# CESSProject/DeOSS

Measured on AMD Instinct MI355X. Metric: device-resident GiB/s hashed to Merkle root; 1/2/4/8 MI355X scaling, higher is better.
Workload: dtype u32; 1 GPU; BASELINE configs[1]: 1 object of 8 GiB (8589934592 B) in 1 chunk-range shard(s) of 8 GiB, chunk 33554432 B (256 leaves); object_bytes=8589934592, chunk=33554432, leaves=256, parallelism=single GPU

## Files before the change

deoss_amd/csrc/merkle_kernels.hpp:

```cpp
#pragma once
#include "quad_ring.hpp"
#include "sha256_gfx950.hpp"

namespace dm {

constexpr int kBlock = 256;
constexpr int kLeafFuseMax = 8;
constexpr int kReduceTile = 512;

struct LeafArgs {
    const uint8_t* base;
    uint64_t pitch;
    uint64_t leaf_len;
    uint64_t last_len;
    const uint64_t* addrs;
    const uint64_t* lens;
    uint64_t nleaves;
    uint64_t byte_off;
    uint64_t byte_end;
    uint32_t* state;
    uint8_t* digests;
    uint8_t* level_out;
    uint32_t fuse_levels;
};
// ... 398 lines not shown
    const uint64_t first = (uint64_t)blockIdx.x * kPairLeaves;
    const uint64_t i = first + c;
    const LeafView v = leaf_view<TABLE>(a, i);
    const uint64_t NB = wave_max_u64(v.nb);
    if (producer) {
        Blk cur;
        if (v.nb > 0 && !lane_b) cur = load_block<ALIGNED>(v.p);
        for (uint64_t b = 0; b < NB; b++) {
            if (b < v.nb) {
                uint32_t w[16];
                block_words(cur, w);
                if (b + 1 < v.nb && !lane_b) cur = load_block<ALIGNED>(v.p + 64 * (b + 1));
                uint4 (*kw)[kLatLeaves] = ring[b % kLatRing];
#pragma unroll
                for (int q = 0; q < 16; q++) {
                    uint32_t u[4];
#pragma unroll
                    for (int j = 0; j < 4; j++) {
                        const int t = 4 * q + j;
                        uint32_t wt;
                        if (t < 16) {
                            wt = w[t];
                        } else {
                            wt = ssig1(w[(t - 2) & 15]) + w[(t - 7) & 15] + ssig0(w[(t - 15) & 15]) + w[t & 15];
                            w[t & 15] = wt;
                        }
                        u[j] = lane_b ? 0u : kSha256K[t] + wt;
                    }
                    kw[q][lane] = make_uint4(u[0], u[1], u[2], u[3]);
                }
            }
            __syncthreads();
        }
        __syncthreads();
    } else {
        const uint32_t sh1 = lane_b ? 2 : 6, sh2 = lane_b ? 13 : 11, sh3 = lane_b ? 22 : 25;
        const uint32_t msk = lane_b ? 0u : ~0u;
        uint32_t st0[8];
        if (v.active) load_or_init_state(a, i, st0);
        else init_state(st0);
        uint32_t x[4];
#pragma unroll
        for (int k = 0; k < 4; k++) x[k] = lane_b ? st0[k] : st0[4 + k];
        __syncthreads();
        for (uint64_t b = 0; b < NB; b++) {
            if (b < v.nb) pair_rounds_from_kw(x, ring[b % kLatRing], lane, sh1, sh2, sh3, msk, lane_b);
            __syncthreads();
        }
        uint32_t st[8];
#pragma unroll
        for (int k = 0; k < 4; k++) {
            const uint32_t other = dpp_swap_pairs(x[k]);
            st[k] = lane_b ? x[k] : other;
            st[4 + k] = lane_b ? other : x[k];
        }
        if (v.active && !lane_b) {
            leaf_epilogue<ALIGNED>(a, i, v, st);
#pragma unroll
            for (int k = 0; k < 8; k++) lds_a[c][k] = st[k];
        }
    }
    if (a.fuse_levels == 0) return;
    __syncthreads();
    const uint32_t cnt = (uint32_t)((a.nleaves - first) < kPairLeaves ? (a.nleaves - first) : kPairLeaves);
    uint32_t (*res)[8];
    const uint32_t out_cnt = lds_reduce(lds_a, lds_b, cnt, a.fuse_levels, &res);
    if (threadIdx.x < out_cnt) {
        uint32_t o8[8];
#pragma unroll
        for (int k = 0; k < 8; k++) o8[k] = res[threadIdx.x][k];
        const uint64_t o = (uint64_t)blockIdx.x * (kPairLeaves >> a.fuse_levels) + threadIdx.x;
        store_digest(a.level_out + 32 * o, o8);
    }
}

constexpr int kQuadLeaves = 8;
constexpr int kQuadBlocks = 8;
constexpr int kQuadFuseMax = 3;
constexpr int kQuadRow = kQuadLeaves;
constexpr size_t kQuadLdsBytes = sizeof(uint4) * kLatRing * 16 * kQuadBlocks * kQuadRow + 4 * 8 * kQuadLeaves +
                                 4 * 8 * (kQuadLeaves / 2);
static_assert(4 * kQuadLdsBytes <= (160u << 10), "four compact K1Q workgroups must fit a CU's LDS");

#define DM_QS_HEAD(X4, X5, X6)                                                                   \
    "v_alignbit_b32 %[r], %[" X4 "], %[" X4 "], %[sh]\n\t"                                      \
    "v_bitop3_b32 %[f], %[" X4 "], %[" X5 "], %[msk] bitop3:0x1e\n\t"                          \
    "v_bitop3_b32 %[f], %[f], %[" X6 "], %[" X5 "] bitop3:0xca\n\t"                             \
    "v_xor_b32_dpp %[s], %[r], %[r] quad_perm:[1,2,0,3] row_mask:0xf bank_mask:0xf\n\t"
#define DM_QS_SIGMA "v_xor_b32_dpp %[s], %[r], %[s] quad_perm:[2,0,1,3] row_mask:0xf bank_mask:0xf\n\t"
#define DM_QS_STEP_Q(X4, X5, X6, X7, H, HN, VN, QP)                                             \
    DM_QS_HEAD(X4, X5, X6)                                                                       \
    "v_sub_u32_dpp %[" X6 "], %[" VN "], %[" X6 "] quad_perm:" QP " row_mask:0xf bank_mask:0x3\n\t" \
    DM_QS_SIGMA                                                                                  \
    "v_sub_u32_dpp %[" HN "], %[" X4 "], %[" X6 "] row_ror:8 row_mask:0xf bank_mask:0xf\n\t"    \
    "v_add3_u32 %[" X7 "], %[s], %[f], %[" H "]\n\t"
#define DM_QS_STEP(X4, X5, X6, X7, H, HN, VN) DM_QS_STEP_Q(X4, X5, X6, X7, H, HN, VN, "[0,1,2,3]")
#define DM_QS_STEP_A(X4, X5, X6, X7, H, HN)                                                     \
    DM_QS_HEAD(X4, X5, X6)                                                                       \
    DM_QS_SIGMA                                                                                  \
    "v_sub_u32_dpp %[" HN "], %[" X4 "], %[" X6 "] row_ror:8 row_mask:0xf bank_mask:0xf\n\t"    \
    "v_add3_u32 %[" X7 "], %[s], %[f], %[" H "]\n\t"
#define DM_QS_STEP_END(X4, X5, X6, X7, H)                                                       \
    DM_QS_HEAD(X4, X5, X6)                                                                       \
    DM_QS_SIGMA                                                                                  \
    "v_add3_u32 %[" X7 "], %[s], %[f], %[" H "]\n\t"
#define DM_QS_STEPS4V(V0, V1, V2, V3)                                                          \
    DM_QS_STEP("a", "b", "c", "d", "h", "g", V0) DM_QS_STEP("d", "a", "b", "c", "g", "h", V1)   \
    DM_QS_STEP("c", "d", "a", "b", "h", "g", V2) DM_QS_STEP("b", "c", "d", "a", "g", "h", V3)
#define DM_QS_ALIGN_MIS ".p2align 3\n\t.if %[mis]\n\ts_nop 0\n\t.endif\n\t"
#define DM_QS_PROLOGUE(V) DM_QS_PROLOGUE_AT(V, DM_QS_ALIGN_MIS, "[0,1,2,3]")
#define DM_QS_PROLOGUE_AT(V, ALIGN, QP)                                                           \
    "s_nop 1\n\t" ALIGN                                                                          \
    "v_sub_u32_dpp %[d], %[" V "], %[d] quad_perm:" QP " row_mask:0xf bank_mask:0x3\n\t"         \
    "v_sub_u32_dpp %[h], %[b], %[d] row_ror:8 row_mask:0xf bank_mask:0xf\n\t"
#define DM_QS_RESTORE_A(P, X) "v_mov_b32_dpp %[" P "], %[" X "] quad_perm:[0,1,2,3] row_mask:0xf bank_mask:0xc\n\t"
#define DM_QS_GROUP0(V0, V1, V2, V3)                                                             \
    DM_QS_STEP("a", "b", "c", "d", "h", "g", V0) DM_QS_RESTORE_A("d", "x3")                      \
    DM_QS_STEP("d", "a", "b", "c", "g", "h", V1) DM_QS_RESTORE_A("c", "x2")                      \
    DM_QS_STEP("c", "d", "a", "b", "h", "g", V2) DM_QS_STEP("b", "c", "d", "a", "g", "h", V3)
#define DM_QS_FF(X, P, BANKS) "v_add_u32_dpp %[" X "], %[" P "], %[" X "] quad_perm:[0,1,2,3] row_mask:0xf bank_mask:" BANKS "\n\t"
#define DM_QS_TAIL(V0, V1, V2)                                                                   \
    DM_QS_STEP("a", "b", "c", "d", "h", "g", V0) DM_QS_STEP("d", "a", "b", "c", "g", "h", V1)   \
    DM_QS_STEP("c", "d", "a", "b", "h", "g", V2) DM_QS_STEP_A("b", "c", "d", "a", "g", "h")      \
    DM_QS_FF("x3", "d", "0x3") DM_QS_FF("x2", "c", "0x3") DM_QS_FF("x1", "b", "0x3")             \
    DM_QS_FF("x0", "a", "0x3")                                                                   \
    DM_QS_STEP_A("a", "b", "c", "d", "h", "g") DM_QS_STEP_END("d", "a", "b", "c", "g")           \
    DM_QS_FF("x0", "a", "0xc") DM_QS_FF("x1", "b", "0xc") DM_QS_FF("x3", "d", "0xc")             \
    DM_QS_FF("x2", "c", "0xc")
#define DM_QS_STEPS4Q(V0, Q0, V1, Q1, V2, Q2, V3, Q3)                                          \
    DM_QS_STEP_Q("a", "b", "c", "d", "h", "g", V0, Q0) DM_QS_STEP_Q("d", "a", "b", "c", "g", "h", V1, Q1) \
    DM_QS_STEP_Q("c", "d", "a", "b", "h", "g", V2, Q2) DM_QS_STEP_Q("b", "c", "d", "a", "g", "h", V3, Q3)
#define DM_QS_GROUP0Q(V0, Q0, V1, Q1, V2, Q2, V3, Q3)                                          \
    DM_QS_STEP_Q("a", "b", "c", "d", "h", "g", V0, Q0) DM_QS_RESTORE_A("d", "x3")              \
    DM_QS_STEP_Q("d", "a", "b", "c", "g", "h", V1, Q1) DM_QS_RESTORE_A("c", "x2")              \
    DM_QS_STEP_Q("c", "d", "a", "b", "h", "g", V2, Q2) DM_QS_STEP_Q("b", "c", "d", "a", "g", "h", V3, Q3)
#define DM_QS_TAILQ(V0, Q0, V1, Q1, V2, Q2)                                                     \
    DM_QS_STEP_Q("a", "b", "c", "d", "h", "g", V0, Q0) DM_QS_STEP_Q("d", "a", "b", "c", "g", "h", V1, Q1) \
    DM_QS_STEP_Q("c", "d", "a", "b", "h", "g", V2, Q2) DM_QS_STEP_A("b", "c", "d", "a", "g", "h") \
    DM_QS_FF("x3", "d", "0x3") DM_QS_FF("x2", "c", "0x3") DM_QS_FF("x1", "b", "0x3")             \
    DM_QS_FF("x0", "a", "0x3")                                                                   \
    DM_QS_STEP_A("a", "b", "c", "d", "h", "g") DM_QS_STEP_END("d", "a", "b", "c", "g")           \
    DM_QS_FF("x0", "a", "0xc") DM_QS_FF("x1", "b", "0xc") DM_QS_FF("x3", "d", "0xc")             \
    DM_QS_FF("x2", "c", "0xc")
#define DM_QS_OUT                                                                                \
    : [a] "+v"(p0), [b] "+v"(p1), [c] "+v"(p2), [d] "+v"(p3), [h] "+v"(h), [g] "+v"(g),           \
      [x0] "+v"(x[0]), [x1] "+v"(x[1]), [x2] "+v"(x[2]), [x3] "+v"(x[3]), [r] "=&v"(r_),          \
      [f] "=&v"(f_), [s] "=&v"(s_)
#define DM_QS_OPS DM_QS_OUT : [mis] "i"(MIS ? 1 : 0), [sh] "v"(sh.x), [msk] "v"(msk), [v0] "v"(v0), [v1] "v"(v1), [v2] "v"(v2), [v3] "v"(v3)

template <bool MIS, class KW>
__device__ __forceinline__ void quad_block_skewed(uint32_t (&x)[4], KW kw, uint3 sh, uint32_t msk) {
    uint32_t p0 = x[0], p1 = x[1], p2 = x[2], p3 = x[3], h = 0, g = 0, r_, f_, s_;
    uint4 q = kw(0), nq = kw(1);
    {
        const uint32_t v0 = q.x, v1 = 0, v2 = 0, v3 = 0;
        asm volatile(DM_QS_PROLOGUE("v0") DM_QS_OPS);
    }
#pragma unroll
    for (int grp = 0; grp < 16; grp++) {
        const uint4 nnq = grp + 2 < 16 ? kw(grp + 2) : nq;
        const uint32_t v0 = q.y, v1 = q.z, v2 = q.w, v3 = nq.x;
        if (grp == 0) {
            asm volatile(DM_QS_ALIGN_MIS DM_QS_GROUP0("v0", "v1", "v2", "v3") DM_QS_OPS);
        } else if (grp < 15) {
            asm volatile(DM_QS_ALIGN_MIS DM_QS_STEPS4V("v0", "v1", "v2", "v3") DM_QS_OPS);
        } else {
            asm volatile(DM_QS_ALIGN_MIS DM_QS_TAIL("v0", "v1", "v2") DM_QS_OPS);
        }
        q = nq;
        nq = nnq;
    }
}

constexpr int kLgkmWait0 = 0xC07F;

#define DM_QS_HNB(HN, A, B, BANKS) "v_sub_u32_dpp %[" HN "], %[" A "], %[" B "] row_ror:8 row_mask:0xf bank_mask:" BANKS "\n\t"
#define DM_QS_ADDB(D, A, B, BANKS) "v_add_u32_dpp %[" D "], %[" A "], %[" B "] quad_perm:[0,1,2,3] row_mask:0xf bank_mask:" BANKS "\n\t"
#define DM_QS_MOVB(D, S, BANKS) "v_mov_b32_dpp %[" D "], %[" S "] quad_perm:[0,1,2,3] row_mask:0xf bank_mask:" BANKS "\n\t"
#define DM_QS_KWN(X6, S, N) "v_sub_u32_dpp %[" X6 "], %[" N "], %[" S "] quad_perm:[0,0,0,0] row_mask:0xf bank_mask:0x3\n\t"
#define DM_QS_ADD3(X7, H) "v_add3_u32 %[" X7 "], %[s], %[f], %[" H "]\n\t"
#define DM_QS_LINKQ(V0, Q0, V1, Q1, V2, Q2, N0, N1, N2)                                          \
    DM_QS_STEP_Q("a", "b", "c", "d", "h", "g", V0, Q0) DM_QS_STEP_Q("d", "a", "b", "c", "g", "h", V1, Q1) \
    DM_QS_STEP_Q("c", "d", "a", "b", "h", "g", V2, Q2)                                           \
    DM_QS_ADDB("x1", "x1", "b", "0xc") DM_QS_ADDB("x3", "x3", "d", "0x3")                        \
                                            \
    DM_QS_HEAD("b", "c", "d") DM_QS_KWN("d", "x3", N0) DM_QS_SIGMA                               \
    DM_QS_HNB("h", "x1", "d", "0x3") DM_QS_HNB("h", "b", "d", "0xc") DM_QS_ADD3("a", "g")        \
    DM_QS_ADDB("b", "x1", "b", "0x3") DM_QS_ADDB("c", "x2", "c", "0x3")                          \
    DM_QS_HNB("g", "a", "c", "0xc") DM_QS_ADDB("x0", "x0", "a", "0xc")                           \
    DM_QS_ADDB("a", "a", "x0", "0x3") DM_QS_MOVB("x2", "c", "0x3")                               \
                                                            \
    DM_QS_HEAD("a", "b", "c") DM_QS_KWN("c", "c", N1) DM_QS_SIGMA                                \
    DM_QS_HNB("g", "x0", "c", "0x3") DM_QS_ADD3("d", "h")                                        \
    DM_QS_ADDB("x3", "x3", "d", "0xc") DM_QS_MOVB("x1", "b", "0x3") DM_QS_MOVB("x0", "a", "0x3") \
                                           \
    DM_QS_HEAD("d", "a", "b") DM_QS_KWN("b", "b", N2) DM_QS_SIGMA                                \
    DM_QS_HNB("h", "x3", "b", "0x3") DM_QS_HNB("h", "d", "x1", "0xc") DM_QS_ADD3("c", "g")       \
    DM_QS_ADDB("x2", "x2", "c", "0xc") DM_QS_MOVB("a", "x0", "0xc") DM_QS_MOVB("d", "x3", "0xc") \
    DM_QS_MOVB("c", "x2", "0xc")
#define DM_QS_BODYQ                                                                              \
    DM_QS_STEPS4Q("q01", "[1,1,1,1]", "q02", "[1,1,1,1]", "q03", "[1,1,1,1]", "q00", "[2,2,2,2]") \
    DM_QS_STEPS4Q("q01", "[2,2,2,2]", "q02", "[2,2,2,2]", "q03", "[2,2,2,2]", "q00", "[3,3,3,3]") \
    DM_QS_STEPS4Q("q01", "[3,3,3,3]", "q02", "[3,3,3,3]", "q03", "[3,3,3,3]", "q10", "[0,0,0,0]") \
    DM_QS_STEPS4Q("q11", "[0,0,0,0]", "q12", "[0,0,0,0]", "q13", "[0,0,0,0]", "q10", "[1,1,1,1]") \
    DM_QS_STEPS4Q("q11", "[1,1,1,1]", "q12", "[1,1,1,1]", "q13", "[1,1,1,1]", "q10", "[2,2,2,2]") \
    DM_QS_STEPS4Q("q11", "[2,2,2,2]", "q12", "[2,2,2,2]", "q13", "[2,2,2,2]", "q10", "[3,3,3,3]") \
    DM_QS_STEPS4Q("q11", "[3,3,3,3]", "q12", "[3,3,3,3]", "q13", "[3,3,3,3]", "q20", "[0,0,0,0]") \
    DM_QS_STEPS4Q("q21", "[0,0,0,0]", "q22", "[0,0,0,0]", "q23", "[0,0,0,0]", "q20", "[1,1,1,1]") \
    DM_QS_STEPS4Q("q21", "[1,1,1,1]", "q22", "[1,1,1,1]", "q23", "[1,1,1,1]", "q20", "[2,2,2,2]") \
    DM_QS_STEPS4Q("q21", "[2,2,2,2]", "q22", "[2,2,2,2]", "q23", "[2,2,2,2]", "q20", "[3,3,3,3]") \
    DM_QS_STEPS4Q("q21", "[3,3,3,3]", "q22", "[3,3,3,3]", "q23", "[3,3,3,3]", "q30", "[0,0,0,0]") \
    DM_QS_STEPS4Q("q31", "[0,0,0,0]", "q32", "[0,0,0,0]", "q33", "[0,0,0,0]", "q30", "[1,1,1,1]") \
    DM_QS_STEPS4Q("q31", "[1,1,1,1]", "q32", "[1,1,1,1]", "q33", "[1,1,1,1]", "q30", "[2,2,2,2]") \
    DM_QS_STEPS4Q("q31", "[2,2,2,2]", "q32", "[2,2,2,2]", "q33", "[2,2,2,2]", "q30", "[3,3,3,3]")
#define DM_QS_FILLQ                                                                              \
    DM_QS_PROLOGUE_AT("q00", DM_QS_ALIGN_MIS, "[0,0,0,0]")                                       \
    DM_QS_GROUP0Q("q01", "[0,0,0,0]", "q02", "[0,0,0,0]", "q03", "[0,0,0,0]", "q00", "[1,1,1,1]")
#define DM_QS_CONTQ                                                                              \
    DM_QS_ALIGN_MIS                                                                              \
    DM_QS_STEP_Q("c", "d", "a", "b", "h", "g", "q03", "[0,0,0,0]") DM_QS_STEP_Q("b", "c", "d", "a", "g", "h", "q00", "[1,1,1,1]")
#define DM_QS_ENDLINKQ DM_QS_LINKQ("q31", "[3,3,3,3]", "q32", "[3,3,3,3]", "q33", "[3,3,3,3]", "n0", "n1", "n2")
#define DM_QS_ENDTAILQ DM_QS_TAILQ("q31", "[3,3,3,3]", "q32", "[3,3,3,3]", "q33", "[3,3,3,3]")
#define DM_QS_STATE [a] "+v"(P[0]), [b] "+v"(P[1]), [c] "+v"(P[2]), [d] "+v"(P[3]),              \
                    [x0] "+v"(x[0]), [x1] "+v"(x[1]), [x2] "+v"(x[2]), [x3] "+v"(x[3]),           \
                    [r] "=&v"(r_), [f] "=&v"(f_), [s] "=&v"(s_)
#define DM_QS_KIN [mis] "i"(MIS ? 1 : 0), [sh] "v"(sh.x), [msk] "v"(msk),                        \
                  [q00] "v"(K[0].x), [q01] "v"(K[0].y), [q02] "v"(K[0].z), [q03] "v"(K[0].w),     \
                  [q10] "v"(K[1].x), [q11] "v"(K[1].y), [q12] "v"(K[1].z), [q13] "v"(K[1].w),     \
                  [q20] "v"(K[2].x), [q21] "v"(K[2].y), [q22] "v"(K[2].z), [q23] "v"(K[2].w),     \
                  [q30] "v"(K[3].x), [q31] "v"(K[3].y), [q32] "v"(K[3].z), [q33] "v"(K[3].w)

template <bool MIS, int K8>
__device__ __forceinline__ void quad_block_regs(uint32_t (&x)[4], uint32_t (&P)[4], uint32_t& h, uint32_t& g,
                                                const uint4 (&K)[4], const uint4& N, uint3 sh, uint32_t msk) {
    uint32_t r_, f_, s_;
    if constexpr (K8 == 0) {
        asm volatile(DM_QS_FILLQ DM_QS_BODYQ DM_QS_ENDLINKQ
                     : DM_QS_STATE, [h] "=&v"(h), [g] "=&v"(g)
                     : DM_QS_KIN, [n0] "v"(N.x), [n1] "v"(N.y), [n2] "v"(N.z));
    } else if constexpr (K8 < kQuadBlocks - 1) {
        asm volatile(DM_QS_CONTQ DM_QS_BODYQ DM_QS_ENDLINKQ
                     : DM_QS_STATE, [h] "+v"(h), [g] "+v"(g)
                     : DM_QS_KIN, [n0] "v"(N.x), [n1] "v"(N.y), [n2] "v"(N.z));
    } else {
        asm volatile(DM_QS_CONTQ DM_QS_BODYQ DM_QS_ENDTAILQ
                     : DM_QS_STATE, [h] "+v"(h), [g] "+v"(g)
                     : DM_QS_KIN);
    }
}

template <int G, int ROW, bool MIS, int K8 = 0>
__device__ __forceinline__ void quad_stage_blocks(uint32_t (&x)[4], uint32_t (&P)[4], uint32_t& h, uint32_t& g,
                                                  uint4 (&S)[3][4], const uint4* kw, uint3 sh, uint32_t msk) {
    __builtin_amdgcn_s_waitcnt(kLgkmWait0);
    if constexpr (K8 + 2 < kQuadBlocks) {
#pragma unroll
        for (int t = 0; t < 4; t++) S[(K8 + 2) % 3][t] = kw[(K8 + 2) * ROW + 4 * t * G];
    }
    quad_block_regs<MIS, K8>(x, P, h, g, S[K8 % 3], S[(K8 + 1) % 3][0], sh, msk);
    if constexpr (K8 + 1 < kQuadBlocks) quad_stage_blocks<G, ROW, MIS, K8 + 1>(x, P, h, g, S, kw, sh, msk);
}
template <int G, int ROW, bool MIS>
__device__ __forceinline__ void quad_stage_regs(uint32_t (&x)[4], const uint4* kw, uint3 sh, uint32_t msk) {
    uint4 S[3][4];
    uint32_t P[4] = {x[0], x[1], x[2], x[3]}, h, g;
#pragma unroll
    for (int k = 0; k < 2; k++) {
#pragma unroll
        for (int t = 0; t < 4; t++) S[k][t] = kw[k * ROW + 4 * t * G];
    }
    quad_stage_blocks<G, ROW, MIS>(x, P, h, g, S, kw, sh, msk);
}

constexpr int kQuadWideRing = quad_ring::kWideDepth;
constexpr int kQuadSets = quad_ring::kSets;
template <int G, int ROW, int K8, bool FILL, bool TAIL, bool LOAD>
__device__ __forceinline__ void quad_xstage_block(uint32_t (&x)[4], uint32_t (&P)[4], uint32_t& h, uint32_t& g,
                                                  uint4 (&S)[kQuadSets][4], const uint4* src, uint3 sh, uint32_t msk) {
    static_assert((LOAD || !quad_ring::block_prefetches(K8, true)) && (!TAIL || !quad_ring::block_links(K8, true)) &&
                      !(FILL && TAIL) && quad_ring::prefetch_of(K8).block == (K8 + quad_ring::kAhead) % kQuadBlocks,
                  "only the last stage of a run skips a load or drains: quad_ring.hpp");
    __builtin_amdgcn_s_waitcnt(kLgkmWait0);
    if constexpr (LOAD) {
        constexpr quad_ring::BlockRef pf = quad_ring::prefetch_of(K8);
#pragma unroll
        for (int t = 0; t < 4; t++) S[quad_ring::set_of(K8 + quad_ring::kAhead)][t] = src[pf.block * ROW + 4 * t * G];
    }
    quad_block_regs<false, FILL ? 0 : TAIL ? kQuadBlocks - 1 : 1>(x, P, h, g, S[quad_ring::set_of(K8)],
                                                                 S[quad_ring::set_of(K8 + 1)][0], sh, msk);
}
template <int G, int ROW>
__device__ __forceinline__ uint32_t quad_run_xstage(uint32_t (&x)[4], const uint4* colp, uint32_t slot, uint64_t n,
                                                    uint3 sh, uint32_t msk) {
    uint4 S[kQuadSets][4];
    uint32_t P[4] = {x[0], x[1], x[2], x[3]}, h, g;
    const uint4* cur = colp + slot * 16 * G;
#pragma unroll
    for (int k = 0; k < quad_ring::kAhead; k++) {
#pragma unroll
        for (int t = 0; t < 4; t++) S[k][t] = cur[k * ROW + 4 * t * G];
    }
    quad_xstage_block<G, ROW, 0, true, false, true>(x, P, h, g, S, cur, sh, msk);
    for (uint64_t s = 1; s < n; s++) {
        slot = quad_ring::next_slot(slot, kQuadWideRing);
        const uint4* nxt = colp + slot * 16 * G;
        quad_xstage_block<G, ROW, 1, false, false, true>(x, P, h, g, S, cur, sh, msk);
        quad_xstage_block<G, ROW, 2, false, false, true>(x, P, h, g, S, cur, sh, msk);
        quad_xstage_block<G, ROW, 3, false, false, true>(x, P, h, g, S, cur, sh, msk);
        quad_xstage_block<G, ROW, 4, false, false, true>(x, P, h, g, S, cur, sh, msk);
        quad_xstage_block<G, ROW, 5, false, false, true>(x, P, h, g, S, cur, sh, msk);
        quad_xstage_block<G, ROW, 6, false, false, true>(x, P, h, g, S, nxt, sh, msk);
        quad_xstage_block<G, ROW, 7, false, false, true>(x, P, h, g, S, nxt, sh, msk);
        __syncthreads();
        quad_xstage_block<G, ROW, 0, false, false, true>(x, P, h, g, S, nxt, sh, msk);
        cur = nxt;
    }
    quad_xstage_block<G, ROW, 1, false, false, true>(x, P, h, g, S, cur, sh, msk);
    quad_xstage_block<G, ROW, 2, false, false, true>(x, P, h, g, S, cur, sh, msk);
    quad_xstage_block<G, ROW, 3, false, false, true>(x, P, h, g, S, cur, sh, msk);
    quad_xstage_block<G, ROW, 4, false, false, true>(x, P, h, g, S, cur, sh, msk);
    quad_xstage_block<G, ROW, 5, false, false, true>(x, P, h, g, S, cur, sh, msk);
    quad_xstage_block<G, ROW, 6, false, false, false>(x, P, h, g, S, cur, sh, msk);
    quad_xstage_block<G, ROW, 7, false, true, false>(x, P, h, g, S, cur, sh, msk);
    __syncthreads();
    return quad_ring::next_slot(slot, kQuadWideRing);
}

template <bool ALIGNED, int G>
__device__ __forceinline__ void quad_produce_block(const LeafView& v, Blk& cur, uint64_t b, uint4* kw) {
    if (b >= v.nb) return;
    uint32_t w[16];
    block_words(cur, w);
    if (b + kQuadBlocks < v.nb) cur = load_block<ALIGNED>(v.p + 64 * (b + kQuadBlocks));
#pragma unroll
    for (int q = 0; q < 16; q++) {
        uint32_t u[4];
#pragma unroll
        for (int k = 0; k < 4; k++) {
            const int t = 4 * q + k;
            uint32_t wt;
            if (t < 16) {
                wt = w[t];
            } else {
                wt = ssig1(w[(t - 2) & 15]) + w[(t - 7) & 15] + ssig0(w[(t - 15) & 15]) + w[t & 15];
                w[t & 15] = wt;
            }
            u[k] = 0u - (kSha256K[t] + wt);
        }
        kw[q * G] = make_uint4(u[0], u[1], u[2], u[3]);
    }
}

template <bool TABLE, bool ALIGNED, bool COMPACT>
__global__ __launch_bounds__(kLatThreads) void leaf_kernel_quad(LeafArgs a) {
    constexpr int ROW = COMPACT ? kQuadRow : kQuadLeaves;
    constexpr int G = kQuadBlocks * ROW;
    constexpr int DEPTH = COMPACT ? kLatRing : kQuadWideRing;
    __shared__ uint4 ring[COMPACT ? 1 : 2][kLatRing][16][G];
    __shared__ uint32_t lds_a[kQuadLeaves][8];
    __shared__ uint32_t lds_b[kQuadLeaves / 2][8];
    static_assert(DEPTH * sizeof(ring[0][0]) <= sizeof(ring), "the ring's stages must fit its LDS");
    static_assert(COMPACT || (3 * sizeof(ring) > (160u << 10) && sizeof(ring) <= (64u << 10) &&
                              2 * (sizeof(ring) + sizeof(lds_a) + sizeof(lds_b)) <= (160u << 10)),
                  "the wide K1Q must stay at exactly two workgroups per CU (160 KiB of LDS)");
    const uint32_t lane = threadIdx.x & 63;
    const bool producer = __builtin_amdgcn_readfirstlane(threadIdx.x) < 64;
    const uint32_t c = lane >> 3;
    const uint32_t j = lane & 7;
    const uint64_t first = (uint64_t)blockIdx.x * kQuadLeaves;
    const uint64_t i = first + c;
    const LeafView v = leaf_view<TABLE>(a, i);
    const uint64_t NB = wave_max_u64(v.nb);
    const uint64_t NI = (NB + kQuadBlocks - 1) / kQuadBlocks;
    if (producer) {
        Blk cur;
        if (j < v.nb) cur = load_block<ALIGNED>(v.p + 64 * j);
        if constexpr (!COMPACT) {
            uint4* const kw0 = &ring[0][0][0][j * ROW + c];
            uint32_t slot = 0;
            for (uint64_t s = 0; s < quad_ring::stages_before_first_barrier(DEPTH); s++) {
                if (s < NI) quad_produce_block<ALIGNED, G>(v, cur, s * kQuadBlocks + j, kw0 + slot * 16 * G);
                slot = quad_ring::next_slot(slot, DEPTH);
            }
            __syncthreads();
            for (uint64_t it = 0; it < NI; it++) {
                const uint64_t s = quad_ring::stage_written_after_barrier(it, DEPTH);
                if (s < NI) quad_produce_block<ALIGNED, G>(v, cur, s * kQuadBlocks + j, kw0 + slot * 16 * G);
                slot = quad_ring::next_slot(slot, DEPTH);
                __syncthreads();
            }
        } else {
            for (uint64_t it = 0; it < NI; it++) {
                const uint64_t b = it * kQuadBlocks + j;
                if (b < v.nb) {
                    uint32_t w[16];
                    block_words(cur, w);
                    if (b + kQuadBlocks < v.nb) cur = load_block<ALIGNED>(v.p + 64 * (b + kQuadBlocks));
                    uint4* kw = &ring[0][it % kLatRing][0][j * ROW + c];
#pragma unroll
                    for (int q = 0; q < 16; q++) {
                        uint32_t u[4];
#pragma unroll
                        for (int k = 0; k < 4; k++) {
                            const int t = 4 * q + k;
                            uint32_t wt;
                            if (t < 16) {
// ... 216 lines not shown
```

Before: 16.90 GiB/s.

## Rename registers across block boundaries in quad SHA-256 asm to drop feed-forward moves

Reworks the inline-asm SHA-256 quad-lane block chain so that consecutive blocks alternate between two register sets (even/odd variants), with extra scratch registers Y[5]. The feed-forward additions are fused into the link/tail sequences instead of being followed by v_mov_b32_dpp restores. The goal is fewer DPP move instructions and shorter dependency chains per 64-byte block. The cost is five more live VGPRs per thread, which may reduce occupancy, and the hand-scheduled DPP bank-mask logic is fragile.

Result: no change. 17.05 GiB/s, median of 6 (+0.9%).

```diff
diff --git a/deoss_amd/csrc/merkle_kernels.hpp b/deoss_amd/csrc/merkle_kernels.hpp
--- a/deoss_amd/csrc/merkle_kernels.hpp
+++ b/deoss_amd/csrc/merkle_kernels.hpp
@@ -504,11 +504,12 @@
                                  4 * 8 * (kQuadLeaves / 2);
 static_assert(4 * kQuadLdsBytes <= (160u << 10), "four compact K1Q workgroups must fit a CU's LDS");
 
-#define DM_QS_HEAD(X4, X5, X6)                                                                   \
+#define DM_QS_HEAD_F(X4, X5, X6)                                                                 \
     "v_alignbit_b32 %[r], %[" X4 "], %[" X4 "], %[sh]\n\t"                                      \
     "v_bitop3_b32 %[f], %[" X4 "], %[" X5 "], %[msk] bitop3:0x1e\n\t"                          \
-    "v_bitop3_b32 %[f], %[f], %[" X6 "], %[" X5 "] bitop3:0xca\n\t"                             \
-    "v_xor_b32_dpp %[s], %[r], %[r] quad_perm:[1,2,0,3] row_mask:0xf bank_mask:0xf\n\t"
+    "v_bitop3_b32 %[f], %[f], %[" X6 "], %[" X5 "] bitop3:0xca\n\t"
+#define DM_QS_HEAD_S "v_xor_b32_dpp %[s], %[r], %[r] quad_perm:[1,2,0,3] row_mask:0xf bank_mask:0xf\n\t"
+#define DM_QS_HEAD(X4, X5, X6) DM_QS_HEAD_F(X4, X5, X6) DM_QS_HEAD_S
 #define DM_QS_SIGMA "v_xor_b32_dpp %[s], %[r], %[s] quad_perm:[2,0,1,3] row_mask:0xf bank_mask:0xf\n\t"
 #define DM_QS_STEP_Q(X4, X5, X6, X7, H, HN, VN, QP)                                             \
     DM_QS_HEAD(X4, X5, X6)                                                                       \
@@ -549,21 +550,13 @@
     DM_QS_STEP_A("a", "b", "c", "d", "h", "g") DM_QS_STEP_END("d", "a", "b", "c", "g")           \
     DM_QS_FF("x0", "a", "0xc") DM_QS_FF("x1", "b", "0xc") DM_QS_FF("x3", "d", "0xc")             \
     DM_QS_FF("x2", "c", "0xc")
-#define DM_QS_STEPS4Q(V0, Q0, V1, Q1, V2, Q2, V3, Q3)                                          \
-    DM_QS_STEP_Q("a", "b", "c", "d", "h", "g", V0, Q0) DM_QS_STEP_Q("d", "a", "b", "c", "g", "h", V1, Q1) \
-    DM_QS_STEP_Q("c", "d", "a", "b", "h", "g", V2, Q2) DM_QS_STEP_Q("b", "c", "d", "a", "g", "h", V3, Q3)
+#define DM_QS_STEPS4Q(A, B, C, D, V0, Q0, V1, Q1, V2, Q2, V3, Q3)                              \
+    DM_QS_STEP_Q(A, B, C, D, "h", "g", V0, Q0) DM_QS_STEP_Q(D, A, B, C, "g", "h", V1, Q1)       \
+    DM_QS_STEP_Q(C, D, A, B, "h", "g", V2, Q2) DM_QS_STEP_Q(B, C, D, A, "g", "h", V3, Q3)
 #define DM_QS_GROUP0Q(V0, Q0, V1, Q1, V2, Q2, V3, Q3)                                          \
     DM_QS_STEP_Q("a", "b", "c", "d", "h", "g", V0, Q0) DM_QS_RESTORE_A("d", "x3")              \
     DM_QS_STEP_Q("d", "a", "b", "c", "g", "h", V1, Q1) DM_QS_RESTORE_A("c", "x2")              \
     DM_QS_STEP_Q("c", "d", "a", "b", "h", "g", V2, Q2) DM_QS_STEP_Q("b", "c", "d", "a", "g", "h", V3, Q3)
-#define DM_QS_TAILQ(V0, Q0, V1, Q1, V2, Q2)                                                     \
-    DM_QS_STEP_Q("a", "b", "c", "d", "h", "g", V0, Q0) DM_QS_STEP_Q("d", "a", "b", "c", "g", "h", V1, Q1) \
-    DM_QS_STEP_Q("c", "d", "a", "b", "h", "g", V2, Q2) DM_QS_STEP_A("b", "c", "d", "a", "g", "h") \
-    DM_QS_FF("x3", "d", "0x3") DM_QS_FF("x2", "c", "0x3") DM_QS_FF("x1", "b", "0x3")             \
-    DM_QS_FF("x0", "a", "0x3")                                                                   \
-    DM_QS_STEP_A("a", "b", "c", "d", "h", "g") DM_QS_STEP_END("d", "a", "b", "c", "g")           \
-    DM_QS_FF("x0", "a", "0xc") DM_QS_FF("x1", "b", "0xc") DM_QS_FF("x3", "d", "0xc")             \
-    DM_QS_FF("x2", "c", "0xc")
 #define DM_QS_OUT                                                                                \
     : [a] "+v"(p0), [b] "+v"(p1), [c] "+v"(p2), [d] "+v"(p3), [h] "+v"(h), [g] "+v"(g),           \
       [x0] "+v"(x[0]), [x1] "+v"(x[1]), [x2] "+v"(x[2]), [x3] "+v"(x[3]), [r] "=&v"(r_),          \
@@ -598,54 +591,87 @@
 
 #define DM_QS_HNB(HN, A, B, BANKS) "v_sub_u32_dpp %[" HN "], %[" A "], %[" B "] row_ror:8 row_mask:0xf bank_mask:" BANKS "\n\t"
 #define DM_QS_ADDB(D, A, B, BANKS) "v_add_u32_dpp %[" D "], %[" A "], %[" B "] quad_perm:[0,1,2,3] row_mask:0xf bank_mask:" BANKS "\n\t"
-#define DM_QS_MOVB(D, S, BANKS) "v_mov_b32_dpp %[" D "], %[" S "] quad_perm:[0,1,2,3] row_mask:0xf bank_mask:" BANKS "\n\t"
-#define DM_QS_KWN(X6, S, N) "v_sub_u32_dpp %[" X6 "], %[" N "], %[" S "] quad_perm:[0,0,0,0] row_mask:0xf bank_mask:0x3\n\t"
+#define DM_QS_KWT(T, S, V, QP) "v_sub_u32_dpp %[" T "], %[" V "], %[" S "] quad_perm:" QP " row_mask:0xf bank_mask:0x3\n\t"
+#define DM_QS_KWN(T, S, N) DM_QS_KWT(T, S, N, "[0,0,0,0]")
 #define DM_QS_ADD3(X7, H) "v_add3_u32 %[" X7 "], %[s], %[f], %[" H "]\n\t"
-#define DM_QS_LINKQ(V0, Q0, V1, Q1, V2, Q2, N0, N1, N2)                                          \
-    DM_QS_STEP_Q("a", "b", "c", "d", "h", "g", V0, Q0) DM_QS_STEP_Q("d", "a", "b", "c", "g", "h", V1, Q1) \
-    DM_QS_STEP_Q("c", "d", "a", "b", "h", "g", V2, Q2)                                           \
-    DM_QS_ADDB("x1", "x1", "b", "0xc") DM_QS_ADDB("x3", "x3", "d", "0x3")                        \
-                                            \
-    DM_QS_HEAD("b", "c", "d") DM_QS_KWN("d", "x3", N0) DM_QS_SIGMA                               \
-    DM_QS_HNB("h", "x1", "d", "0x3") DM_QS_HNB("h", "b", "d", "0xc") DM_QS_ADD3("a", "g")        \
-    DM_QS_ADDB("b", "x1", "b", "0x3") DM_QS_ADDB("c", "x2", "c", "0x3")                          \
-    DM_QS_HNB("g", "a", "c", "0xc") DM_QS_ADDB("x0", "x0", "a", "0xc")                           \
-    DM_QS_ADDB("a", "a", "x0", "0x3") DM_QS_MOVB("x2", "c", "0x3")                               \
-                                                            \
-    DM_QS_HEAD("a", "b", "c") DM_QS_KWN("c", "c", N1) DM_QS_SIGMA                                \
-    DM_QS_HNB("g", "x0", "c", "0x3") DM_QS_ADD3("d", "h")                                        \
-    DM_QS_ADDB("x3", "x3", "d", "0xc") DM_QS_MOVB("x1", "b", "0x3") DM_QS_MOVB("x0", "a", "0x3") \
-                                           \
-    DM_QS_HEAD("d", "a", "b") DM_QS_KWN("b", "b", N2) DM_QS_SIGMA                                \
-    DM_QS_HNB("h", "x3", "b", "0x3") DM_QS_HNB("h", "d", "x1", "0xc") DM_QS_ADD3("c", "g")       \
-    DM_QS_ADDB("x2", "x2", "c", "0xc") DM_QS_MOVB("a", "x0", "0xc") DM_QS_MOVB("d", "x3", "0xc") \
-    DM_QS_MOVB("c", "x2", "0xc")
-#define DM_QS_BODYQ                                                                              \
-    DM_QS_STEPS4Q("q01", "[1,1,1,1]", "q02", "[1,1,1,1]", "q03", "[1,1,1,1]", "q00", "[2,2,2,2]") \
-    DM_QS_STEPS4Q("q01", "[2,2,2,2]", "q02", "[2,2,2,2]", "q03", "[2,2,2,2]", "q00", "[3,3,3,3]") \
-    DM_QS_STEPS4Q("q01", "[3,3,3,3]", "q02", "[3,3,3,3]", "q03", "[3,3,3,3]", "q10", "[0,0,0,0]") \
-    DM_QS_STEPS4Q("q11", "[0,0,0,0]", "q12", "[0,0,0,0]", "q13", "[0,0,0,0]", "q10", "[1,1,1,1]") \
-    DM_QS_STEPS4Q("q11", "[1,1,1,1]", "q12", "[1,1,1,1]", "q13", "[1,1,1,1]", "q10", "[2,2,2,2]") \
-    DM_QS_STEPS4Q("q11", "[2,2,2,2]", "q12", "[2,2,2,2]", "q13", "[2,2,2,2]", "q10", "[3,3,3,3]") \
-    DM_QS_STEPS4Q("q11", "[3,3,3,3]", "q12", "[3,3,3,3]", "q13", "[3,3,3,3]", "q20", "[0,0,0,0]") \
-    DM_QS_STEPS4Q("q21", "[0,0,0,0]", "q22", "[0,0,0,0]", "q23", "[0,0,0,0]", "q20", "[1,1,1,1]") \
-    DM_QS_STEPS4Q("q21", "[1,1,1,1]", "q22", "[1,1,1,1]", "q23", "[1,1,1,1]", "q20", "[2,2,2,2]") \
-    DM_QS_STEPS4Q("q21", "[2,2,2,2]", "q22", "[2,2,2,2]", "q23", "[2,2,2,2]", "q20", "[3,3,3,3]") \
-    DM_QS_STEPS4Q("q21", "[3,3,3,3]", "q22", "[3,3,3,3]", "q23", "[3,3,3,3]", "q30", "[0,0,0,0]") \
-    DM_QS_STEPS4Q("q31", "[0,0,0,0]", "q32", "[0,0,0,0]", "q33", "[0,0,0,0]", "q30", "[1,1,1,1]") \
-    DM_QS_STEPS4Q("q31", "[1,1,1,1]", "q32", "[1,1,1,1]", "q33", "[1,1,1,1]", "q30", "[2,2,2,2]") \
-    DM_QS_STEPS4Q("q31", "[2,2,2,2]", "q32", "[2,2,2,2]", "q33", "[2,2,2,2]", "q30", "[3,3,3,3]")
+#define DM_QS_LINKQ(W0, W1, W2, W3, Y0, Y1, E0, E1, E2, E3, AA, AB, AC, AD, V0, Q0, V1, Q1, V2, Q2, N0, N1, N2) \
+    DM_QS_STEP_Q(W0, W1, W2, W3, "h", "g", V0, Q0) DM_QS_STEP_Q(W3, W0, W1, W2, "g", "h", V1, Q1) \
+    DM_QS_STEP_Q(W2, W3, W0, W1, "h", "g", V2, Q2)                                               \
+        \
+    DM_QS_HEAD_F(W1, W2, W3) DM_QS_ADDB(W3, E3, W3, "0x3") DM_QS_ADDB("t", AD, W1, "0xc")        \
+    DM_QS_KWN("t", W3, N0) DM_QS_HEAD_S DM_QS_SIGMA                                              \
+    DM_QS_HNB("h", "t", "t", "0x3") DM_QS_HNB("h", W1, W3, "0xc") DM_QS_ADD3(W0, "g")            \
+    DM_QS_ADDB(W1, E1, W1, "0x3") DM_QS_ADDB(W2, E2, W2, "0x3")                                  \
+    DM_QS_HNB("g", W0, W2, "0xc") DM_QS_ADDB(W0, E0, W0, "0x3")                                  \
+                           \
+    DM_QS_HEAD(W0, W1, W2) DM_QS_KWN("t", W2, N1) DM_QS_SIGMA DM_QS_ADD3(Y0, "h")                \
+       \
+    DM_QS_HEAD(Y0, W0, W1) DM_QS_ADDB(W0, AC, W0, "0xc") DM_QS_ADDB(Y0, AB, Y0, "0xc")           \
+    DM_QS_SIGMA DM_QS_HNB("g", W0, "t", "0x3") DM_QS_KWN("t", W1, N2)                            \
+                               \
+    DM_QS_HNB("h", Y0, "t", "0xf") DM_QS_ADD3(Y1, "g")                                           \
+    DM_QS_ADDB(Y1, AA, Y1, "0xc")
+#define DM_QS_TAILQ(W0, W1, W2, W3, Z0, Z1, E0, E1, E2, E3, AA, AB, AC, AD, V0, Q0, V1, Q1, V2, Q2) \
+    DM_QS_STEP_Q(W0, W1, W2, W3, "h", "g", V0, Q0) DM_QS_STEP_Q(W3, W0, W1, W2, "g", "h", V1, Q1) \
+    DM_QS_STEP_Q(W2, W3, W0, W1, "h", "g", V2, Q2) DM_QS_STEP_A(W1, W2, W3, W0, "g", "h")        \
+    DM_QS_ADDB("x3", E3, W3, "0x3") DM_QS_ADDB("x2", E2, W2, "0x3") DM_QS_ADDB("x1", E1, W1, "0x3") \
+              \
+    DM_QS_STEP_A(W0, W1, W2, Z0, "h", "g") DM_QS_ADDB("x0", E0, W0, "0x3")                       \
+    DM_QS_STEP_END(Z0, W0, W1, Z1, "g")                                                          \
+    DM_QS_ADDB("x1", AD, W1, "0xc") DM_QS_ADDB("x0", AC, W0, "0xc") DM_QS_ADDB("x3", AB, Z0, "0xc") \
+    DM_QS_ADDB("x2", AA, Z1, "0xc")
+#define DM_QS_BODYQ(A, B, C, D)                                                                 \
+    DM_QS_STEP_Q(D, A, B, C, "g", "h", "q02", "[1,1,1,1]") DM_QS_STEP_Q(C, D, A, B, "h", "g", "q03", "[1,1,1,1]") \
+    DM_QS_STEP_Q(B, C, D, A, "g", "h", "q00", "[2,2,2,2]")                                       \
+    DM_QS_STEPS4Q(A, B, C, D, "q01", "[2,2,2,2]", "q02", "[2,2,2,2]", "q03", "[2,2,2,2]", "q00", "[3,3,3,3]") \
+    DM_QS_STEPS4Q(A, B, C, D, "q01", "[3,3,3,3]", "q02", "[3,3,3,3]", "q03", "[3,3,3,3]", "q10", "[0,0,0,0]") \
+    DM_QS_STEPS4Q(A, B, C, D, "q11", "[0,0,0,0]", "q12", "[0,0,0,0]", "q13", "[0,0,0,0]", "q10", "[1,1,1,1]") \
+    DM_QS_STEPS4Q(A, B, C, D, "q11", "[1,1,1,1]", "q12", "[1,1,1,1]", "q13", "[1,1,1,1]", "q10", "[2,2,2,2]") \
+    DM_QS_STEPS4Q(A, B, C, D, "q11", "[2,2,2,2]", "q12", "[2,2,2,2]", "q13", "[2,2,2,2]", "q10", "[3,3,3,3]") \
+    DM_QS_STEPS4Q(A, B, C, D, "q11", "[3,3,3,3]", "q12", "[3,3,3,3]", "q13", "[3,3,3,3]", "q20", "[0,0,0,0]") \
+    DM_QS_STEPS4Q(A, B, C, D, "q21", "[0,0,0,0]", "q22", "[0,0,0,0]", "q23", "[0,0,0,0]", "q20", "[1,1,1,1]") \
+    DM_QS_STEPS4Q(A, B, C, D, "q21", "[1,1,1,1]", "q22", "[1,1,1,1]", "q23", "[1,1,1,1]", "q20", "[2,2,2,2]") \
+    DM_QS_STEPS4Q(A, B, C, D, "q21", "[2,2,2,2]", "q22", "[2,2,2,2]", "q23", "[2,2,2,2]", "q20", "[3,3,3,3]") \
+    DM_QS_STEPS4Q(A, B, C, D, "q21", "[3,3,3,3]", "q22", "[3,3,3,3]", "q23", "[3,3,3,3]", "q30", "[0,0,0,0]") \
+    DM_QS_STEPS4Q(A, B, C, D, "q31", "[0,0,0,0]", "q32", "[0,0,0,0]", "q33", "[0,0,0,0]", "q30", "[1,1,1,1]") \
+    DM_QS_STEPS4Q(A, B, C, D, "q31", "[1,1,1,1]", "q32", "[1,1,1,1]", "q33", "[1,1,1,1]", "q30", "[2,2,2,2]") \
+    DM_QS_STEPS4Q(A, B, C, D, "q31", "[2,2,2,2]", "q32", "[2,2,2,2]", "q33", "[2,2,2,2]", "q30", "[3,3,3,3]")
 #define DM_QS_FILLQ                                                                              \
     DM_QS_PROLOGUE_AT("q00", DM_QS_ALIGN_MIS, "[0,0,0,0]")                                       \
-    DM_QS_GROUP0Q("q01", "[0,0,0,0]", "q02", "[0,0,0,0]", "q03", "[0,0,0,0]", "q00", "[1,1,1,1]")
-#define DM_QS_CONTQ                                                                              \
+    DM_QS_GROUP0Q("q01", "[0,0,0,0]", "q02", "[0,0,0,0]", "q03", "[0,0,0,0]", "q00", "[1,1,1,1]") \
+    DM_QS_STEP_Q("a", "b", "c", "d", "h", "g", "q01", "[1,1,1,1]")
+#define DM_QS_CONTQ(W0, Y0, Y1, A, B, C, D)                                                     \
     DM_QS_ALIGN_MIS                                                                              \
-    DM_QS_STEP_Q("c", "d", "a", "b", "h", "g", "q03", "[0,0,0,0]") DM_QS_STEP_Q("b", "c", "d", "a", "g", "h", "q00", "[1,1,1,1]")
-#define DM_QS_ENDLINKQ DM_QS_LINKQ("q31", "[3,3,3,3]", "q32", "[3,3,3,3]", "q33", "[3,3,3,3]", "n0", "n1", "n2")
-#define DM_QS_ENDTAILQ DM_QS_TAILQ("q31", "[3,3,3,3]", "q32", "[3,3,3,3]", "q33", "[3,3,3,3]")
+    DM_QS_HEAD(Y1, Y0, W0) DM_QS_KWT("t", W0, "q03", "[0,0,0,0]") DM_QS_SIGMA                    \
+    DM_QS_HNB("g", Y1, "t", "0x3") DM_QS_HNB("g", Y1, W0, "0xc") DM_QS_ADD3(B, "h")              \
+    DM_QS_STEP_Q(B, Y1, Y0, A, "g", "h", "q00", "[1,1,1,1]")                                     \
+    DM_QS_STEP_Q(A, B, Y1, D, "h", "g", "q01", "[1,1,1,1]")
+#define DM_QS_BODYQ_E DM_QS_BODYQ("a", "b", "c", "d")
+#define DM_QS_BODYQ_O DM_QS_BODYQ("x0", "x1", "x2", "x3")
+#define DM_QS_CONTQ_E DM_QS_CONTQ("x0", "u0", "u1", "a", "b", "c", "d")
+#define DM_QS_CONTQ_O DM_QS_CONTQ("a", "y0", "y1", "x0", "x1", "x2", "x3")
+#define DM_QS_ENDLINKQ_F                                                                         \
+    DM_QS_LINKQ("a", "b", "c", "d", "y0", "y1", "x0", "x1", "x2", "x3", "x2", "x3", "x0", "x1", \
+                 "q31", "[3,3,3,3]", "q32", "[3,3,3,3]", "q33", "[3,3,3,3]", "n0", "n1", "n2")
+#define DM_QS_ENDLINKQ_E                                                                         \
+    DM_QS_LINKQ("a", "b", "c", "d", "y0", "y1", "x0", "x1", "x2", "x3", "u1", "u0", "x0", "t", \
+                 "q31", "[3,3,3,3]", "q32", "[3,3,3,3]", "q33", "[3,3,3,3]", "n0", "n1", "n2")
+#define DM_QS_ENDLINKQ_O                                                                         \
+    DM_QS_LINKQ("x0", "x1", "x2", "x3", "u0", "u1", "a", "b", "c", "d", "y1", "y0", "a", "t", \
+                 "q31", "[3,3,3,3]", "q32", "[3,3,3,3]", "q33", "[3,3,3,3]", "n0", "n1", "n2")
+#define DM_QS_ENDTAILQ_F                                                                         \
+    DM_QS_TAILQ("a", "b", "c", "d", "y0", "y1", "x0", "x1", "x2", "x3", "x2", "x3", "x0", "x1", \
+                 "q31", "[3,3,3,3]", "q32", "[3,3,3,3]", "q33", "[3,3,3,3]")
+#define DM_QS_ENDTAILQ_E                                                                         \
+    DM_QS_TAILQ("a", "b", "c", "d", "y0", "y1", "x0", "x1", "x2", "x3", "u1", "u0", "x0", "t", \
+                 "q31", "[3,3,3,3]", "q32", "[3,3,3,3]", "q33", "[3,3,3,3]")
+#define DM_QS_ENDTAILQ_O                                                                         \
+    DM_QS_TAILQ("x0", "x1", "x2", "x3", "u0", "u1", "a", "b", "c", "d", "y1", "y0", "a", "t", \
+                 "q31", "[3,3,3,3]", "q32", "[3,3,3,3]", "q33", "[3,3,3,3]")
 #define DM_QS_STATE [a] "+v"(P[0]), [b] "+v"(P[1]), [c] "+v"(P[2]), [d] "+v"(P[3]),              \
                     [x0] "+v"(x[0]), [x1] "+v"(x[1]), [x2] "+v"(x[2]), [x3] "+v"(x[3]),           \
-                    [r] "=&v"(r_), [f] "=&v"(f_), [s] "=&v"(s_)
+                    [y0] "+v"(Y[0]), [y1] "+v"(Y[1]), [u0] "+v"(Y[2]), [u1] "+v"(Y[3]),           \
+                    [t] "+v"(Y[4]), [r] "=&v"(r_), [f] "=&v"(f_), [s] "=&v"(s_)
 #define DM_QS_KIN [mis] "i"(MIS ? 1 : 0), [sh] "v"(sh.x), [msk] "v"(msk),                        \
                   [q00] "v"(K[0].x), [q01] "v"(K[0].y), [q02] "v"(K[0].z), [q03] "v"(K[0].w),     \
                   [q10] "v"(K[1].x), [q11] "v"(K[1].y), [q12] "v"(K[1].z), [q13] "v"(K[1].w),     \
@@ -653,52 +679,59 @@
                   [q30] "v"(K[3].x), [q31] "v"(K[3].y), [q32] "v"(K[3].z), [q33] "v"(K[3].w)
 
 template <bool MIS, int K8>
-__device__ __forceinline__ void quad_block_regs(uint32_t (&x)[4], uint32_t (&P)[4], uint32_t& h, uint32_t& g,
-                                                const uint4 (&K)[4], const uint4& N, uint3 sh, uint32_t msk) {
+__device__ __forceinline__ void quad_block_regs(uint32_t (&x)[4], uint32_t (&P)[4], uint32_t (&Y)[5], uint32_t& h,
+                                                uint32_t& g, const uint4 (&K)[4], const uint4& N, uint3 sh,
+                                                uint32_t msk) {
     uint32_t r_, f_, s_;
     if constexpr (K8 == 0) {
-        asm volatile(DM_QS_FILLQ DM_QS_BODYQ DM_QS_ENDLINKQ
+        asm volatile(DM_QS_FILLQ DM_QS_BODYQ_E DM_QS_ENDLINKQ_F
                      : DM_QS_STATE, [h] "=&v"(h), [g] "=&v"(g)
                      : DM_QS_KIN, [n0] "v"(N.x), [n1] "v"(N.y), [n2] "v"(N.z));
-    } else if constexpr (K8 < kQuadBlocks - 1) {
-        asm volatile(DM_QS_CONTQ DM_QS_BODYQ DM_QS_ENDLINKQ
+    } else if constexpr (K8 == kQuadBlocks - 1) {
+        asm volatile(DM_QS_CONTQ_O DM_QS_BODYQ_O DM_QS_ENDTAILQ_O
+                     : DM_QS_STATE, [h] "+v"(h), [g] "+v"(g)
+                     : DM_QS_KIN);
+    } else if constexpr (K8 % 2 == 1) {
+        asm volatile(DM_QS_CONTQ_O DM_QS_BODYQ_O DM_QS_ENDLINKQ_O
                      : DM_QS_STATE, [h] "+v"(h), [g] "+v"(g)
                      : DM_QS_KIN, [n0] "v"(N.x), [n1] "v"(N.y), [n2] "v"(N.z));
     } else {
-        asm volatile(DM_QS_CONTQ DM_QS_BODYQ DM_QS_ENDTAILQ
+        asm volatile(DM_QS_CONTQ_E DM_QS_BODYQ_E DM_QS_ENDLINKQ_E
                      : DM_QS_STATE, [h] "+v"(h), [g] "+v"(g)
-                     : DM_QS_KIN);
+                     : DM_QS_KIN, [n0] "v"(N.x), [n1] "v"(N.y), [n2] "v"(N.z));
     }
 }
 
 template <int G, int ROW, bool MIS, int K8 = 0>
-__device__ __forceinline__ void quad_stage_blocks(uint32_t (&x)[4], uint32_t (&P)[4], uint32_t& h, uint32_t& g,
-                                                  uint4 (&S)[3][4], const uint4* kw, uint3 sh, uint32_t msk) {
+__device__ __forceinline__ void quad_stage_blocks(uint32_t (&x)[4], uint32_t (&P)[4], uint32_t (&Y)[5], uint32_t& h,
+                                                  uint32_t& g, uint4 (&S)[3][4], const uint4* kw, uint3 sh,
+                                                  uint32_t msk) {
     __builtin_amdgcn_s_waitcnt(kLgkmWait0);
     if constexpr (K8 + 2 < kQuadBlocks) {
 #pragma unroll
         for (int t = 0; t < 4; t++) S[(K8 + 2) % 3][t] = kw[(K8 + 2) * ROW + 4 * t * G];
     }
-    quad_block_regs<MIS, K8>(x, P, h, g, S[K8 % 3], S[(K8 + 1) % 3][0], sh, msk);
-    if constexpr (K8 + 1 < kQuadBlocks) quad_stage_blocks<G, ROW, MIS, K8 + 1>(x, P, h, g, S, kw, sh, msk);
+    quad_block_regs<MIS, K8>(x, P, Y, h, g, S[K8 % 3], S[(K8 + 1) % 3][0], sh, msk);
+    if constexpr (K8 + 1 < kQuadBlocks) quad_stage_blocks<G, ROW, MIS, K8 + 1>(x, P, Y, h, g, S, kw, sh, msk);
 }
 template <int G, int ROW, bool MIS>
 __device__ __forceinline__ void quad_stage_regs(uint32_t (&x)[4], const uint4* kw, uint3 sh, uint32_t msk) {
     uint4 S[3][4];
-    uint32_t P[4] = {x[0], x[1], x[2], x[3]}, h, g;
+    uint32_t P[4] = {x[0], x[1], x[2], x[3]}, Y[5] = {0, 0, 0, 0, 0}, h, g;
 #pragma unroll
     for (int k = 0; k < 2; k++) {
 #pragma unroll
         for (int t = 0; t < 4; t++) S[k][t] = kw[k * ROW + 4 * t * G];
     }
-    quad_stage_blocks<G, ROW, MIS>(x, P, h, g, S, kw, sh, msk);
+    quad_stage_blocks<G, ROW, MIS>(x, P, Y, h, g, S, kw, sh, msk);
 }
 
 constexpr int kQuadWideRing = quad_ring::kWideDepth;
 constexpr int kQuadSets = quad_ring::kSets;
 template <int G, int ROW, int K8, bool FILL, bool TAIL, bool LOAD>
-__device__ __forceinline__ void quad_xstage_block(uint32_t (&x)[4], uint32_t (&P)[4], uint32_t& h, uint32_t& g,
-                                                  uint4 (&S)[kQuadSets][4], const uint4* src, uint3 sh, uint32_t msk) {
+__device__ __forceinline__ void quad_xstage_block(uint32_t (&x)[4], uint32_t (&P)[4], uint32_t (&Y)[5], uint32_t& h,
+                                                  uint32_t& g, uint4 (&S)[kQuadSets][4], const uint4* src, uint3 sh,
+                                                  uint32_t msk) {
     static_assert((LOAD || !quad_ring::block_prefetches(K8, true)) && (!TAIL || !quad_ring::block_links(K8, true)) &&
                       !(FILL && TAIL) && quad_ring::prefetch_of(K8).block == (K8 + quad_ring::kAhead) % kQuadBlocks,
                   "only the last stage of a run skips a load or drains: quad_ring.hpp");
@@ -708,42 +741,42 @@
 #pragma unroll
         for (int t = 0; t < 4; t++) S[quad_ring::set_of(K8 + quad_ring::kAhead)][t] = src[pf.block * ROW + 4 * t * G];
     }
-    quad_block_regs<false, FILL ? 0 : TAIL ? kQuadBlocks - 1 : 1>(x, P, h, g, S[quad_ring::set_of(K8)],
-                                                                 S[quad_ring::set_of(K8 + 1)][0], sh, msk);
+    quad_block_regs<false, FILL ? 0 : TAIL ? kQuadBlocks - 1 : K8 % 2 ? 1 : 2>(
+        x, P, Y, h, g, S[quad_ring::set_of(K8)], S[quad_ring::set_of(K8 + 1)][0], sh, msk);
 }
 template <int G, int ROW>
 __device__ __forceinline__ uint32_t quad_run_xstage(uint32_t (&x)[4], const uint4* colp, uint32_t slot, uint64_t n,
                                                     uint3 sh, uint32_t msk) {
     uint4 S[kQuadSets][4];
-    uint32_t P[4] = {x[0], x[1], x[2], x[3]}, h, g;
+    uint32_t P[4] = {x[0], x[1], x[2], x[3]}, Y[5] = {0, 0, 0, 0, 0}, h, g;
     const uint4* cur = colp + slot * 16 * G;
 #pragma unroll
     for (int k = 0; k < quad_ring::kAhead; k++) {
 #pragma unroll
         for (int t = 0; t < 4; t++) S[k][t] = cur[k * ROW + 4 * t * G];
     }
-    quad_xstage_block<G, ROW, 0, true, false, true>(x, P, h, g, S, cur, sh, msk);
+    quad_xstage_block<G, ROW, 0, true, false, true>(x, P, Y, h, g, S, cur, sh, msk);
     for (uint64_t s = 1; s < n; s++) {
         slot = quad_ring::next_slot(slot, kQuadWideRing);
         const uint4* nxt = colp + slot * 16 * G;
-        quad_xstage_block<G, ROW, 1, false, false, true>(x, P, h, g, S, cur, sh, msk);
-        quad_xstage_block<G, ROW, 2, false, false, true>(x, P, h, g, S, cur, sh, msk);
-        quad_xstage_block<G, ROW, 3, false, false, true>(x, P, h, g, S, cur, sh, msk);
-        quad_xstage_block<G, ROW, 4, false, false, true>(x, P, h, g, S, cur, sh, msk);
-        quad_xstage_block<G, ROW, 5, false, false, true>(x, P, h, g, S, cur, sh, msk);
-        quad_xstage_block<G, ROW, 6, false, false, true>(x, P, h, g, S, nxt, sh, msk);
-        quad_xstage_block<G, ROW, 7, false, false, true>(x, P, h, g, S, nxt, sh, msk);
+        quad_xstage_block<G, ROW, 1, false, false, true>(x, P, Y, h, g, S, cur, sh, msk);
+        quad_xstage_block<G, ROW, 2, false, false, true>(x, P, Y, h, g, S, cur, sh, msk);
+        quad_xstage_block<G, ROW, 3, false, false, true>(x, P, Y, h, g, S, cur, sh, msk);
+        quad_xstage_block<G, ROW, 4, false, false, true>(x, P, Y, h, g, S, cur, sh, msk);
+        quad_xstage_block<G, ROW, 5, false, false, true>(x, P, Y, h, g, S, cur, sh, msk);
+        quad_xstage_block<G, ROW, 6, false, false, true>(x, P, Y, h, g, S, nxt, sh, msk);
+        quad_xstage_block<G, ROW, 7, false, false, true>(x, P, Y, h, g, S, nxt, sh, msk);
         __syncthreads();
-        quad_xstage_block<G, ROW, 0, false, false, true>(x, P, h, g, S, nxt, sh, msk);
+        quad_xstage_block<G, ROW, 0, false, false, true>(x, P, Y, h, g, S, nxt, sh, msk);
         cur = nxt;
     }
-    quad_xstage_block<G, ROW, 1, false, false, true>(x, P, h, g, S, cur, sh, msk);
-    quad_xstage_block<G, ROW, 2, false, false, true>(x, P, h, g, S, cur, sh, msk);
-    quad_xstage_block<G, ROW, 3, false, false, true>(x, P, h, g, S, cur, sh, msk);
-    quad_xstage_block<G, ROW, 4, false, false, true>(x, P, h, g, S, cur, sh, msk);
-    quad_xstage_block<G, ROW, 5, false, false, true>(x, P, h, g, S, cur, sh, msk);
-    quad_xstage_block<G, ROW, 6, false, false, false>(x, P, h, g, S, cur, sh, msk);
-    quad_xstage_block<G, ROW, 7, false, true, false>(x, P, h, g, S, cur, sh, msk);
+    quad_xstage_block<G, ROW, 1, false, false, true>(x, P, Y, h, g, S, cur, sh, msk);
+    quad_xstage_block<G, ROW, 2, false, false, true>(x, P, Y, h, g, S, cur, sh, msk);
+    quad_xstage_block<G, ROW, 3, false, false, true>(x, P, Y, h, g, S, cur, sh, msk);
+    quad_xstage_block<G, ROW, 4, false, false, true>(x, P, Y, h, g, S, cur, sh, msk);
+    quad_xstage_block<G, ROW, 5, false, false, true>(x, P, Y, h, g, S, cur, sh, msk);
+    quad_xstage_block<G, ROW, 6, false, false, false>(x, P, Y, h, g, S, cur, sh, msk);
+    quad_xstage_block<G, ROW, 7, false, true, false>(x, P, Y, h, g, S, cur, sh, msk);
     __syncthreads();
     return quad_ring::next_slot(slot, kQuadWideRing);
 }
```
